# fengweie/UDA_CLR

Hardware: AMD Instinct MI355X
Metric: training images/sec (512x512, src+tgt) at 1/2/4/8 MI355X; val Dice vs ref (higher is better)
Workload: dtype f32

## Files before the change

uda_clr_amd/csrc/dwconv.hip:

```cpp
#include "dw_plan.h"

struct DwArgs {
    uda_src_t src;
    const float* w9c;
    int stride, dil, border_mode;
    int Ho, Wo;
    float* y;
    int64_t ldy;
    const float* dy;
    int64_t lddy;
    float* part;
    double* stats;
};

__device__ __forceinline__ float4 dw_transform(float4 v, const Xf4& xf, bool has_xf, int act) {
    float r[4] = {v.x, v.y, v.z, v.w};
#pragma unroll
    for (int j = 0; j < 4; ++j) {
        float u = r[j];
        if (has_xf) u = u * xf.sc[j] + xf.sh[j];
        r[j] = uda_act(u, act);
    }
    return make_float4(r[0], r[1], r[2], r[3]);
}

__global__ __launch_bounds__(256) void dwconv_fwd_kernel(DwArgs a) {
    __shared__ float red[2 * 1024];
    const int C = a.src.C, G = C >> 2, PP = 256 / G;
    const int tid = threadIdx.x, cg = tid % G, pl = tid / G;
    const bool active = pl < PP;
    const int H = a.src.H, W = a.src.W;
    const int64_t Pout = (int64_t)a.src.N * a.Ho * a.Wo;
    const int c0 = cg * 4;
    const bool has_xf = a.src.scale != nullptr;
    const int act = a.src.act;
    Xf4 xf;
    uda_load_xf4(xf, a.src.scale, a.src.shift, c0, C);
    float4 bval = make_float4(0.f, 0.f, 0.f, 0.f);
    if (a.border_mode == 1)
        bval = make_float4(uda_act(xf.sh[0], act), uda_act(xf.sh[1], act), uda_act(xf.sh[2], act), uda_act(xf.sh[3], act));
    float4 w[9];
#pragma unroll
    for (int t = 0; t < 9; ++t) w[t] = active ? uda_ld4(a.w9c + t * C + c0) : make_float4(0.f, 0.f, 0.f, 0.f);
    float4 s1 = make_float4(0.f, 0.f, 0.f, 0.f), s2 = s1;
    const int64_t base = (int64_t)blockIdx.x * (PP * DW_ITER_FWD);
    for (int it = 0; it < DW_ITER_FWD; ++it) {
        const int64_t po = base + (int64_t)it * PP + pl;
        if (!active || po >= Pout) continue;
        const int ow = (int)(po % a.Wo), oh = (int)((po / a.Wo) % a.Ho), n = (int)(po / ((int64_t)a.Wo * a.Ho));
        float4 acc = make_float4(0.f, 0.f, 0.f, 0.f);
#pragma unroll
        for (int kh = 0; kh < 3; ++kh) {
            const int ih = oh * a.stride + (kh - 1) * a.dil;
#pragma unroll
            for (int kw = 0; kw < 3; ++kw) {
                const int iw = ow * a.stride + (kw - 1) * a.dil;
                float4 u = bval;
                if (ih >= 0 && ih < H && iw >= 0 && iw < W)
                    u = dw_transform(uda_ld4(a.src.x + (((int64_t)n * H + ih) * W + iw) * a.src.ldx + c0), xf, has_xf, act);
                const float4 ww = w[kh * 3 + kw];
                acc.x += ww.x * u.x; acc.y += ww.y * u.y; acc.z += ww.z * u.z; acc.w += ww.w * u.w;
            }
        }
        uda_st4(a.y + po * a.ldy + c0, acc);
        s1.x += acc.x; s1.y += acc.y; s1.z += acc.z; s1.w += acc.w;
        s2.x += acc.x * acc.x; s2.y += acc.y * acc.y; s2.z += acc.z * acc.z; s2.w += acc.w * acc.w;
    }
    if (a.stats == nullptr) return;
    if (active) {
        uda_st4(&red[(pl * 2 + 0) * C + c0], s1);
        uda_st4(&red[(pl * 2 + 1) * C + c0], s2);
    }
    __syncthreads();
    double* dst = a.stats + (int64_t)(blockIdx.x % UDA_STAT_SLOTS) * 2 * C;
    for (int e = tid; e < 2 * C; e += 256) {
        float t = 0.f;
        for (int p = 0; p < PP; ++p) t += red[p * 2 * C + e];
        atomicAdd(&dst[e], (double)t);
    }
}

template <int S, int TH, int TW>
__device__ __forceinline__ void dw_stage_tile(float* tile, const float* xb, int64_t ldx, int H, int W, int gy0, int gx0, int IH, int IW, bool cok,
                                              const Xf4& xf, bool has_xf, int act, float4 bval, int pl, int cg) {
    constexpr int MAXL = (((TH - 1) * S + 5) * ((TW - 1) * S + 5) + 31) / 32;
    float4 v[MAXL];
    const int npix = IH * IW;
#pragma unroll
    for (int l = 0; l < MAXL; ++l) {
        const int idx = min(pl + 32 * l, npix - 1);
        const int iy = idx / IW, ix = idx - iy * IW;
        const int gy = min(max(gy0 + iy, 0), H - 1), gx = min(max(gx0 + ix, 0), W - 1);
        v[l] = uda_ld4(xb + ((int64_t)gy * W + gx) * ldx);
    }
#pragma unroll
    for (int l = 0; l < MAXL; ++l) {
        const int idx = pl + 32 * l;
        if (idx < npix) {
            const int iy = idx / IW, ix = idx - iy * IW;
            const int gy = gy0 + iy, gx = gx0 + ix;
            const bool in = cok && gy >= 0 && gy < H && gx >= 0 && gx < W;
            const float4 u = in ? dw_transform(v[l], xf, has_xf, act) : bval;
            uda_st4(&tile[idx * DWT_CB + cg * 4], u);
        }
    }
}

template <int S, int TH, int TW>
__global__ __launch_bounds__(256) void dwconv_fwd_tiled_kernel(DwArgs a, int tilesX, int tilesY) {
    extern __shared__ __attribute__((aligned(16))) float tile[];
    const int d = a.dil;
    const int IH = (TH - 1) * S + 2 * d + 1, IW = (TW - 1) * S + 2 * d + 1;
    const int C = a.src.C, H = a.src.H, W = a.src.W;
    const int tid = threadIdx.x, cg = tid & 7, pl = tid >> 3;
    int bt = blockIdx.x;
    const int tx = bt % tilesX; bt /= tilesX;
    const int ty = bt % tilesY;
    const int n = bt / tilesY;
    const int oy0 = ty * TH, ox0 = tx * TW;
    const int c0 = blockIdx.y * DWT_CB + cg * 4;
    const bool cok = c0 < C;
    const bool has_xf = a.src.scale != nullptr;
    const int act = a.src.act;
    Xf4 xf;
    uda_load_xf4(xf, a.src.scale, a.src.shift, c0, C);
    float4 bval = make_float4(0.f, 0.f, 0.f, 0.f);
    if (a.border_mode == 1)
        bval = make_float4(uda_act(xf.sh[0], act), uda_act(xf.sh[1], act), uda_act(xf.sh[2], act), uda_act(xf.sh[3], act));
    const int gy0 = oy0 * S - d, gx0 = ox0 * S - d;
    const float* xb = a.src.x + (int64_t)n * H * W * a.src.ldx + (cok ? c0 : 0);
    dw_stage_tile<S, TH, TW>(tile, xb, a.src.ldx, H, W, gy0, gx0, IH, IW, cok, xf, has_xf, act, bval, pl, cg);
    float4 w[9];
#pragma unroll
    for (int t = 0; t < 9; ++t) w[t] = cok ? uda_ld4(a.w9c + t * C + c0) : make_float4(0.f, 0.f, 0.f, 0.f);
    __syncthreads();
    float4 s1 = make_float4(0.f, 0.f, 0.f, 0.f), s2 = s1;
#pragma unroll
    for (int k = 0; k < (TH * TW) / 32; ++k) {
        const int op = pl + 32 * k;
        const int oy = op / TW, ox = op % TW;
        if (!cok || oy0 + oy >= a.Ho || ox0 + ox >= a.Wo) continue;
        float4 acc = make_float4(0.f, 0.f, 0.f, 0.f);
#pragma unroll
        for (int kh = 0; kh < 3; ++kh)
#pragma unroll
            for (int kw = 0; kw < 3; ++kw) {
                const float4 u = uda_ld4(&tile[((oy * S + kh * d) * IW + ox * S + kw * d) * DWT_CB + cg * 4]);
                const float4 ww = w[kh * 3 + kw];
                acc.x += ww.x * u.x; acc.y += ww.y * u.y; acc.z += ww.z * u.z; acc.w += ww.w * u.w;
            }
        uda_st4(a.y + (((int64_t)n * a.Ho + oy0 + oy) * a.Wo + ox0 + ox) * a.ldy + c0, acc);
        s1.x += acc.x; s1.y += acc.y; s1.z += acc.z; s1.w += acc.w;
        s2.x += acc.x * acc.x; s2.y += acc.y * acc.y; s2.z += acc.z * acc.z; s2.w += acc.w * acc.w;
    }
    if (a.stats == nullptr) return;
    __syncthreads();
    uda_st4(&tile[(pl * 2 + 0) * DWT_CB + cg * 4], s1);
    uda_st4(&tile[(pl * 2 + 1) * DWT_CB + cg * 4], s2);
    __syncthreads();
    if (tid < 2 * DWT_CB) {
        const int q = tid / DWT_CB, cl = tid % DWT_CB;
        const int c = blockIdx.y * DWT_CB + cl;
        if (c < C) {
            float t = 0.f;
            for (int p = 0; p < 32; ++p) t += tile[(p * 2 + q) * DWT_CB + cl];
            atomicAdd(&a.stats[((int64_t)(blockIdx.x % UDA_STAT_SLOTS) * 2 + q) * C + c], (double)t);
        }
    }
}

template <int S, int TH, int TW>
__global__ __launch_bounds__(256) void dwconv_wgrad_tiled_kernel(DwArgs a, int tilesX, int tilesY, double* sums) {
    extern __shared__ __attribute__((aligned(16))) float tile[];
    const int d = a.dil;
    const int IH = (TH - 1) * S + 2 * d + 1, IW = (TW - 1) * S + 2 * d + 1;
    const int C = a.src.C, H = a.src.H, W = a.src.W;
    const int tid = threadIdx.x, cg = tid & 7, pl = tid >> 3;
    int bt = blockIdx.x;
    const int tx = bt % tilesX; bt /= tilesX;
    const int ty = bt % tilesY;
    const int n = bt / tilesY;
    const int oy0 = ty * TH, ox0 = tx * TW;
    const int c0 = blockIdx.y * DWT_CB + cg * 4;
    const bool cok = c0 < C;
    const bool has_xf = a.src.scale != nullptr;
    const int act = a.src.act;
    Xf4 xf;
    uda_load_xf4(xf, a.src.scale, a.src.shift, c0, C);
    float4 bval = make_float4(0.f, 0.f, 0.f, 0.f);
    if (a.border_mode == 1)
        bval = make_float4(uda_act(xf.sh[0], act), uda_act(xf.sh[1], act), uda_act(xf.sh[2], act), uda_act(xf.sh[3], act));
    const int gy0 = oy0 * S - d, gx0 = ox0 * S - d;
    const float* xb = a.src.x + (int64_t)n * H * W * a.src.ldx + (cok ? c0 : 0);
    dw_stage_tile<S, TH, TW>(tile, xb, a.src.ldx, H, W, gy0, gx0, IH, IW, cok, xf, has_xf, act, bval, pl, cg);
    __syncthreads();
    float4 acc[9];
#pragma unroll
    for (int t = 0; t < 9; ++t) acc[t] = make_float4(0.f, 0.f, 0.f, 0.f);
    float4 gv[(TH * TW) / 32];
#pragma unroll
    for (int k = 0; k < (TH * TW) / 32; ++k) {
        const int op = pl + 32 * k;
        const int oy = min(oy0 + op / TW, a.Ho - 1), ox = min(ox0 + op % TW, a.Wo - 1);
        gv[k] = uda_ld4(a.dy + (((int64_t)n * a.Ho + oy) * a.Wo + ox) * a.lddy + (cok ? c0 : 0));
    }
#pragma unroll
    for (int k = 0; k < (TH * TW) / 32; ++k) {
        const int op = pl + 32 * k;
        const int oy = op / TW, ox = op % TW;
        if (!cok || oy0 + oy >= a.Ho || ox0 + ox >= a.Wo) continue;
        const float4 g = gv[k];
#pragma unroll
        for (int kh = 0; kh < 3; ++kh)
#pragma unroll
            for (int kw = 0; kw < 3; ++kw) {
                const float4 u = uda_ld4(&tile[((oy * S + kh * d) * IW + ox * S + kw * d) * DWT_CB + cg * 4]);
                float4& s = acc[kh * 3 + kw];
                s.x += g.x * u.x; s.y += g.y * u.y; s.z += g.z * u.z; s.w += g.w * u.w;
            }
    }
    __syncthreads();
#pragma unroll
    for (int t = 0; t < 9; ++t) uda_st4(&tile[(pl * 9 + t) * DWT_CB + cg * 4], acc[t]);
    __syncthreads();
    for (int e = tid; e < 9 * DWT_CB; e += 256) {
        const int t = e / DWT_CB, cl = e % DWT_CB;
        const int c = blockIdx.y * DWT_CB + cl;
        if (c < C) {
            float v = 0.f;
            for (int p = 0; p < 32; ++p) v += tile[(p * 9 + t) * DWT_CB + cl];
            atomicAdd(&sums[((int64_t)(blockIdx.x % UDA_STAT_SLOTS) * 9 + t) * C + c], (double)v);
        }
    }
}

__global__ void dw_wgrad_store_slots_kernel(const double* __restrict__ sums, int C, float* __restrict__ dw) {
    const int e = blockIdx.x * blockDim.x + threadIdx.x;
    if (e < 9 * C) {
        double v = 0.0;
        for (int k = 0; k < UDA_STAT_SLOTS; ++k) v += sums[(int64_t)k * 9 * C + e];
        dw[(e % C) * 9 + e / C] = (float)v;
    }
}

template <int S, int TH, int TW>
static int launch_dw_tiled(const DwArgs& a, const DwPlan& p, hipStream_t st) {
    auto fn = dwconv_fwd_tiled_kernel<S, TH, TW>;
    static size_t reserved = 0;
    if (p.lds > reserved && p.lds > 48 * 1024) {
        hipError_t e = hipFuncSetAttribute(reinterpret_cast<const void*>(fn), hipFuncAttributeMaxDynamicSharedMemorySize, (int)p.lds);
        if (e != hipSuccess) return uda_set_error("dwconv_fwd: cannot reserve %zu B of LDS: %s", p.lds, hipGetErrorString(e));
        reserved = p.lds;
    }
    hipLaunchKernelGGL(fn, dim3(p.gx, p.gy), dim3(256), p.lds, st, a, p.tilesX, p.tilesY);
    UDA_LAUNCH_CHECK("dwconv_fwd_tiled");
    return 0;
}

template <int S, int TH, int TW>
static int launch_dw_wgrad_tiled(const DwArgs& a, const DwPlan& p, double* sums, hipStream_t st) {
    auto fn = dwconv_wgrad_tiled_kernel<S, TH, TW>;
    static size_t reserved = 0;
    if (p.lds > reserved && p.lds > 48 * 1024) {
        hipError_t e = hipFuncSetAttribute(reinterpret_cast<const void*>(fn), hipFuncAttributeMaxDynamicSharedMemorySize, (int)p.lds);
        if (e != hipSuccess) return uda_set_error("dwconv_wgrad: cannot reserve %zu B of LDS: %s", p.lds, hipGetErrorString(e));
        reserved = p.lds;
    }
    hipLaunchKernelGGL(fn, dim3(p.gx, p.gy), dim3(256), p.lds, st, a, p.tilesX, p.tilesY, sums);
    UDA_LAUNCH_CHECK("dwconv_wgrad_tiled");
    return 0;
}

__global__ __launch_bounds__(256) void dwconv_dgrad_kernel(const float* __restrict__ dy, int64_t lddy,
                                                            const float* __restrict__ w9c, int C, int stride,
                                                            int dil, int N, int H, int W, int Ho, int Wo,
                                                            float* __restrict__ dx, int64_t lddx) {
    const int G = C >> 2;
    const int64_t total = (int64_t)N * H * W * G;
    for (int64_t e = (int64_t)blockIdx.x * blockDim.x + threadIdx.x; e < total; e += (int64_t)gridDim.x * blockDim.x) {
        const int cg = (int)(e % G);
        const int64_t p = e / G;
        const int iw = (int)(p % W), ih = (int)((p / W) % H), n = (int)(p / ((int64_t)W * H));
        const int c0 = cg * 4;
        float4 acc = make_float4(0.f, 0.f, 0.f, 0.f);
        if (stride == 2 && dil == 1) {
            const int khA = (ih & 1) ? 0 : 1, ohA = (ih + 1) >> 1, ohB = (ih - 1) >> 1;
            const int kwA = (iw & 1) ? 0 : 1, owA = (iw + 1) >> 1, owB = (iw - 1) >> 1;
            const int oha = (ih & 1) ? ohA : (ih >> 1), owa = (iw & 1) ? owA : (iw >> 1);
            const bool hA = oha < Ho, hB = (ih & 1) && ohB >= 0 && ohB < Ho;
            const bool wA = owa < Wo, wB = (iw & 1) && owB >= 0 && owB < Wo;
            const int r0 = min(oha, Ho - 1), r1 = min(max(ohB, 0), Ho - 1), q0 = min(owa, Wo - 1), q1 = min(max(owB, 0), Wo - 1);
            const float* base = dy + (int64_t)n * Ho * Wo * lddy + c0;
            const float4 g00 = uda_ld4(base + ((int64_t)r0 * Wo + q0) * lddy), g01 = uda_ld4(base + ((int64_t)r0 * Wo + q1) * lddy);
            const float4 g10 = uda_ld4(base + ((int64_t)r1 * Wo + q0) * lddy), g11 = uda_ld4(base + ((int64_t)r1 * Wo + q1) * lddy);
            const float4 w00 = uda_ld4(w9c + (khA * 3 + kwA) * C + c0), w01 = uda_ld4(w9c + (khA * 3 + 2) * C + c0);
            const float4 w10 = uda_ld4(w9c + (2 * 3 + kwA) * C + c0), w11 = uda_ld4(w9c + (2 * 3 + 2) * C + c0);
            const float k00 = (hA && wA) ? 1.f : 0.f, k01 = (hA && wB) ? 1.f : 0.f, k10 = (hB && wA) ? 1.f : 0.f, k11 = (hB && wB) ? 1.f : 0.f;
            acc.x = k00 * (w00.x * g00.x); acc.y = k00 * (w00.y * g00.y); acc.z = k00 * (w00.z * g00.z); acc.w = k00 * (w00.w * g00.w);
            acc.x += k01 * (w01.x * g01.x); acc.y += k01 * (w01.y * g01.y); acc.z += k01 * (w01.z * g01.z); acc.w += k01 * (w01.w * g01.w);
            acc.x += k10 * (w10.x * g10.x); acc.y += k10 * (w10.y * g10.y); acc.z += k10 * (w10.z * g10.z); acc.w += k10 * (w10.w * g10.w);
            acc.x += k11 * (w11.x * g11.x); acc.y += k11 * (w11.y * g11.y); acc.z += k11 * (w11.z * g11.z); acc.w += k11 * (w11.w * g11.w);
            uda_st4(dx + p * lddx + c0, acc);
            continue;
        }
#pragma unroll
        for (int kh = 0; kh < 3; ++kh) {
            const int nh = ih - (kh - 1) * dil;
            if (nh < 0 || nh % stride) continue;
            const int oh = nh / stride;
            if (oh >= Ho) continue;
#pragma unroll
            for (int kw = 0; kw < 3; ++kw) {
                const int nw = iw - (kw - 1) * dil;
                if (nw < 0 || nw % stride) continue;
                const int ow = nw / stride;
                if (ow >= Wo) continue;
                const float4 g = uda_ld4(dy + (((int64_t)n * Ho + oh) * Wo + ow) * lddy + c0);
                const float4 ww = uda_ld4(w9c + (kh * 3 + kw) * C + c0);
                acc.x += ww.x * g.x; acc.y += ww.y * g.y; acc.z += ww.z * g.z; acc.w += ww.w * g.w;
            }
        }
        uda_st4(dx + p * lddx + c0, acc);
    }
}

__global__ __launch_bounds__(256) void dwconv_wgrad_kernel(DwArgs a) {
    __shared__ float red[9 * 1024];
    const int C = a.src.C, G = C >> 2, PP = 256 / G;
    const int tid = threadIdx.x, cg = tid % G, pl = tid / G;
    const bool active = pl < PP;
    const int H = a.src.H, W = a.src.W;
    const int64_t Pout = (int64_t)a.src.N * a.Ho * a.Wo;
    const int c0 = cg * 4;
    const bool has_xf = a.src.scale != nullptr;
    const int act = a.src.act;
    Xf4 xf;
    uda_load_xf4(xf, a.src.scale, a.src.shift, c0, C);
    float4 bval = make_float4(0.f, 0.f, 0.f, 0.f);
    if (a.border_mode == 1)
        bval = make_float4(uda_act(xf.sh[0], act), uda_act(xf.sh[1], act), uda_act(xf.sh[2], act), uda_act(xf.sh[3], act));
    float4 acc[9];
#pragma unroll
    for (int t = 0; t < 9; ++t) acc[t] = make_float4(0.f, 0.f, 0.f, 0.f);
    const int64_t base = (int64_t)blockIdx.x * (PP * DW_ITER_RED);
// ... 156 lines not shown
#pragma unroll
    for (int t = 0; t < 9; ++t) uda_st4(&red[((pl * 9 + t) * CG + cl) * 4], acc[t]);
    __syncthreads();
    double* dst = sums + (int64_t)(blockIdx.x % UDA_STAT_SLOTS) * 9 * C;
    for (int e = tid; e < 9 * CG * 4; e += 256) {
        const int t = e / (CG * 4), cc = e - t * (CG * 4);
        const int c = blockIdx.y * CG * 4 + cc;
        if (c >= C) continue;
        float v = 0.f;
        for (int p = 0; p < PL; ++p) v += red[(p * 9 + t) * CG * 4 + cc];
        atomicAdd(&dst[t * C + c], (double)v);
    }
}

__global__ __launch_bounds__(256) void dwconv_cb_dgrad_kernel(const float* __restrict__ dy, int64_t lddy,
                                                               const float* __restrict__ w9c, int C, int stride, int dil,
                                                               int N, int H, int W, int Ho, int Wo,
                                                               float* __restrict__ dx, int64_t lddx, int lg) {
    const int CG = 1 << lg, PL = 256 >> lg, G = C >> 2;
    const int tid = threadIdx.x, cl = tid & (CG - 1), pl = tid >> lg;
    const int cg = blockIdx.y * CG + cl;
    const bool cok = cg < G;
    const int c0 = (cok ? cg : G - 1) * 4;
    const int64_t P = (int64_t)N * H * W;
    float4 w[9];
#pragma unroll
    for (int t = 0; t < 9; ++t) w[t] = uda_ld4(w9c + t * C + c0);
    const int64_t base = (int64_t)blockIdx.x * PL * DWB_ITER_FWD;
    for (int it = 0; it < DWB_ITER_FWD; ++it) {
        const int64_t p = base + (int64_t)it * PL + pl;
        if (p >= P) break;
        int n, ih, iw;
        dwb_pixel(p, W, H, n, ih, iw);
        int oh[3], ow[3];
        bool vh[3], vw[3];
#pragma unroll
        for (int k = 0; k < 3; ++k) {
            const int nh = ih - (k - 1) * dil, nw = iw - (k - 1) * dil;
            vh[k] = nh >= 0 && nh % stride == 0 && nh / stride < Ho;
            vw[k] = nw >= 0 && nw % stride == 0 && nw / stride < Wo;
            oh[k] = vh[k] ? nh / stride : 0;
            ow[k] = vw[k] ? nw / stride : 0;
        }
        const float* base_n = dy + (int64_t)n * Ho * Wo * lddy + c0;
        float4 g[9];
#pragma unroll
        for (int kh = 0; kh < 3; ++kh)
#pragma unroll
            for (int kw = 0; kw < 3; ++kw) g[kh * 3 + kw] = uda_ld4(base_n + ((int64_t)oh[kh] * Wo + ow[kw]) * lddy);
        float4 acc = make_float4(0.f, 0.f, 0.f, 0.f);
#pragma unroll
        for (int kh = 0; kh < 3; ++kh)
#pragma unroll
            for (int kw = 0; kw < 3; ++kw) {
                if (!(vh[kh] && vw[kw])) continue;
                const float4 ww = w[kh * 3 + kw], gg = g[kh * 3 + kw];
                acc.x += ww.x * gg.x; acc.y += ww.y * gg.y; acc.z += ww.z * gg.z; acc.w += ww.w * gg.w;
            }
        if (cok) uda_st4(dx + p * lddx + c0, acc);
    }
}

static_assert(DWF_AUTO == UDA_DW_AUTO && DWF_FLAT == UDA_DW_FLAT && DWF_TILED == UDA_DW_TILED && DWF_CB == UDA_DW_CB, "DwFamily is the ABI's UDA_DW_*");
static_assert(DW_FWD == UDA_DW_FWD && DW_DGRAD == UDA_DW_DGRAD && DW_WGRAD == UDA_DW_WGRAD, "DwOp is the ABI's UDA_DW_FWD ...");

static int dw_check(const uda_src_t* s, const char* who) {
    UDA_REQUIRE(s && s->x && uda_aligned16(s->x) && s->ldx % 4 == 0 && s->ldx >= s->C, "%s: bad src", who);
    UDA_REQUIRE((s->scale == nullptr) == (s->shift == nullptr), "%s: scale/shift must come together", who);
    UDA_REQUIRE(s->mask == nullptr, "%s: dropout masks are not supported on depthwise inputs", who);
    return 0;
}

#define DW_REQUIRE_PLAN(p, who, C, stride, dil) UDA_REQUIRE(!(p).error, "%s: C=%d, stride %d, dilation %d: %s", who, C, stride, dil, (p).error)

static DwArgs dw_args(const uda_src_t* src, const DwPlan& p, int stride, int dil, int border_mode) {
    DwArgs a = {};
    a.src = *src;
    a.stride = stride; a.dil = dil; a.border_mode = border_mode;
    a.Ho = p.Ho; a.Wo = p.Wo;
    return a;
}

static int dw_fwd_tiled(const DwArgs& a, const DwPlan& p, hipStream_t st) {
#define DW_LAUNCH(S_, TH_, TW_) if (p.S == S_ && p.TH == TH_ && p.TW == TW_) return launch_dw_tiled<S_, TH_, TW_>(a, p, st);
    DW_TILED_VARIANTS(DW_LAUNCH)
#undef DW_LAUNCH
    return uda_set_error("dwconv_fwd: no tiled kernel <%d, %d, %d>", p.S, p.TH, p.TW);
}

static int dw_wgrad_tiled(const DwArgs& a, const DwPlan& p, double* sums, hipStream_t st) {
#define DW_LAUNCH(S_, TH_, TW_) if (p.S == S_ && p.TH == TH_ && p.TW == TW_) return launch_dw_wgrad_tiled<S_, TH_, TW_>(a, p, sums, st);
    DW_TILED_VARIANTS(DW_LAUNCH)
#undef DW_LAUNCH
    return uda_set_error("dwconv_wgrad: no tiled kernel <%d, %d, %d>", p.S, p.TH, p.TW);
}

extern "C" uint64_t uda_dwconv_workspace_bytes(int64_t Pout, int C) {
    if (C < 4) return 0;
    uint64_t most = 0;
    for (int f = DWF_FLAT; f <= DWF_CB; ++f)
        if (C <= dw_cmax(DW_WGRAD, f)) {
            const uint64_t b = dw_wgrad_ws_bytes(f, Pout, C);
            if (b > most) most = b;
        }
    return most;
}

extern "C" int uda_dwconv_fwd(const uda_src_t* src, const float* w9c, int stride, int dil, int border_mode,
                              float* y, int64_t ldy, double* stats, int family, void* stream) {
    hipStream_t st = (hipStream_t)stream;
    if (int e = dw_check(src, "uda_dwconv_fwd")) return e;
    const DwPlan p = dw_plan(DW_FWD, src->N, src->H, src->W, src->C, stride, dil, family);
    DW_REQUIRE_PLAN(p, "uda_dwconv_fwd", src->C, stride, dil);
    UDA_REQUIRE(w9c && uda_aligned16(w9c) && y && uda_aligned16(y) && ldy % 4 == 0 && ldy >= src->C, "uda_dwconv_fwd: bad pointers");
    UDA_REQUIRE(border_mode == 0 || (border_mode == 1 && src->shift), "uda_dwconv_fwd: border_mode 1 needs shift");
    DwArgs a = dw_args(src, p, stride, dil, border_mode);
    a.w9c = w9c; a.y = y; a.ldy = ldy; a.stats = stats;
    if (p.family == DWF_TILED) return dw_fwd_tiled(a, p, st);
    if (p.family == DWF_CB) hipLaunchKernelGGL(dwconv_cb_fwd_kernel, dim3(p.gx, p.gy), dim3(256), 0, st, a, p.lg);
    else hipLaunchKernelGGL(dwconv_fwd_kernel, dim3(p.gx), dim3(256), 0, st, a);
    UDA_LAUNCH_CHECK(p.family == DWF_CB ? "dwconv_cb_fwd" : "dwconv_fwd");
    return 0;
}

extern "C" int uda_dwconv_dgrad(const float* dy, int64_t lddy, const float* w9c, int C, int stride, int dil,
                                int N, int H, int W, float* dx, int64_t lddx, int family, void* stream) {
    hipStream_t st = (hipStream_t)stream;
    UDA_REQUIRE(dy && w9c && dx && uda_aligned16(dy) && uda_aligned16(dx) && uda_aligned16(w9c), "uda_dwconv_dgrad: pointers must be 16-byte aligned");
    const DwPlan p = dw_plan(DW_DGRAD, N, H, W, C, stride, dil, family);
    DW_REQUIRE_PLAN(p, "uda_dwconv_dgrad", C, stride, dil);
    UDA_REQUIRE(lddy % 4 == 0 && lddx % 4 == 0 && lddy >= C && lddx >= C, "uda_dwconv_dgrad: lds must be multiples of 4, at least C");
    if (p.family == DWF_CB)
        hipLaunchKernelGGL(dwconv_cb_dgrad_kernel, dim3(p.gx, p.gy), dim3(256), 0, st, dy, lddy, w9c, C, stride, dil, N, H, W, p.Ho, p.Wo, dx, lddx, p.lg);
    else
        hipLaunchKernelGGL(dwconv_dgrad_kernel, dim3(p.gx), dim3(256), 0, st, dy, lddy, w9c, C, stride, dil, N, H, W, p.Ho, p.Wo, dx, lddx);
    UDA_LAUNCH_CHECK(p.family == DWF_CB ? "dwconv_cb_dgrad" : "dwconv_dgrad");
    return 0;
}

extern "C" int uda_dwconv_wgrad(const uda_src_t* src, const float* dy, int64_t lddy, int stride, int dil,
                                int border_mode, float* dw, float* workspace, uint64_t workspace_bytes, int family, void* stream) {
    hipStream_t st = (hipStream_t)stream;
    if (int e = dw_check(src, "uda_dwconv_wgrad")) return e;
    const int C = src->C;
    const DwPlan p = dw_plan(DW_WGRAD, src->N, src->H, src->W, C, stride, dil, family);
    DW_REQUIRE_PLAN(p, "uda_dwconv_wgrad", C, stride, dil);
    UDA_REQUIRE(dy && uda_aligned16(dy) && lddy % 4 == 0 && lddy >= C && dw, "uda_dwconv_wgrad: bad pointers");
    UDA_REQUIRE(border_mode == 0 || (border_mode == 1 && src->shift), "uda_dwconv_wgrad: border_mode 1 needs shift");
    UDA_REQUIRE(workspace && workspace_bytes >= uda_dwconv_workspace_bytes(p.Pout, C), "uda_dwconv_wgrad: workspace too small");
    DwArgs a = dw_args(src, p, stride, dil, border_mode);
    a.dy = dy; a.lddy = lddy;
    const dim3 store_grid(uda_cdiv(9 * C, 256));
    if (p.family == DWF_FLAT) {
        a.part = uda_wgp_part(workspace, 9 * C);
        uda_wgp_zero(workspace, 9 * C, st);
        hipLaunchKernelGGL(dwconv_wgrad_kernel, dim3(p.gx), dim3(256), 0, st, a);
        UDA_LAUNCH_CHECK("dwconv_wgrad");
        if (int e = uda_wgp_reduce(workspace, p.part_rows, 9 * C, st)) return e;
        hipLaunchKernelGGL(dw_wgrad_store_kernel, store_grid, dim3(256), 0, st, uda_wgp_sums(workspace), C, dw);
        UDA_LAUNCH_CHECK("dw_wgrad_store");
        return 0;
    }
    double* sums = reinterpret_cast<double*>(workspace);
    (void)hipMemsetAsync(sums, 0, (size_t)p.sum_slots * 9 * C * sizeof(double), st);
    if (p.family == DWF_CB) {
        hipLaunchKernelGGL(dwconv_cb_wgrad_kernel, dim3(p.gx, p.gy), dim3(256), 0, st, a, p.lg, sums);
        UDA_LAUNCH_CHECK("dwconv_cb_wgrad");
    } else if (int e = dw_wgrad_tiled(a, p, sums, st)) return e;
    hipLaunchKernelGGL(dw_wgrad_store_slots_kernel, store_grid, dim3(256), 0, st, sums, C, dw);
    UDA_LAUNCH_CHECK("dw_wgrad_store");
    return 0;
}

static const char* const DW_OP_NAME[3] = {"fwd", "dgrad", "wgrad"};
// ... 261 lines not shown
```

uda_clr_amd/csrc/igemm_conv.hip:

```cpp
#include <algorithm>
#include "common.h"
#include "conv_plan.h"

typedef float f32x16 __attribute__((ext_vector_type(16)));


#define IGC_MIN_WAVES(TM, TN, PIPE) ((PIPE) ? 2 : ((TM) * (TN) <= 3 ? 4 : 3))
template <int TM, int TN, int WM, int WN, bool PIPE = false, int XF = -1>
__global__ __launch_bounds__(256) void igemm_conv_kernel(ConvKArgs a) {
    constexpr int BM = 32 * TM * WM, BN = 32 * TN * WN;
    constexpr int A_IT = BM / 32, B_IT = BN / 32;
    constexpr int TILE = (BM + BN) * IG_LD;
    extern __shared__ __attribute__((aligned(16))) float smem[];

    const int tid = threadIdx.x, lane = tid & 63, wave = tid >> 6;
    const int wm = wave / WN, wn = wave % WN;
    const int lid = uda_xcd_remap(blockIdx.x, a.nMt * a.nNt);
    const int mt = lid / a.nNt, nt = lid % a.nNt;
    const int H = a.src.H, W = a.src.W, C = a.src.C;
    const int64_t P = (int64_t)a.src.N * H * W;
    const int64_t m0 = (int64_t)mt * BM;
    const int n0 = nt * BN;

    const int lrow = tid >> 3, kv = (tid & 7) * 4;
// ... 118 lines not shown
            t01 = f32x2{__builtin_amdgcn_fmed3f(t01.x, alo, ahi), __builtin_amdgcn_fmed3f(t01.y, alo, ahi)};
            t23 = f32x2{__builtin_amdgcn_fmed3f(t23.x, alo, ahi), __builtin_amdgcn_fmed3f(t23.y, alo, ahi)};
            if (masked) {
                const uint32_t mk = amask[i];
                t01 *= f32x2{(float)(mk & 0xffu), (float)((mk >> 8) & 0xffu)} * ms;
                t23 *= f32x2{(float)((mk >> 16) & 0xffu), (float)(mk >> 24)} * ms;
            }
            float v[4] = {t01.x, t01.y, t23.x, t23.y};
#pragma unroll
            for (int j = 0; j < 4; ++j)
                if (!(ok && (c_ci + j) < C)) v[j] = 0.f;
            uda_st4(&As[(lrow + 32 * i) * IG_LD + kv], make_float4(v[0], v[1], v[2], v[3]));
        }
#pragma unroll
        for (int i = 0; i < B_IT; ++i) uda_st4(&Bs[(lrow + 32 * i) * IG_LD + kv], breg[i]);
    };

    f32x16 acc[TM][TN];
#pragma unroll
    for (int i = 0; i < TM; ++i)
#pragma unroll
        for (int j = 0; j < TN; ++j)
#pragma unroll
            for (int r = 0; r < 16; ++r) acc[i][j][r] = 0.f;

    const int nchunks = (a.Ktot + IG_BK - 1) / IG_BK;
    const int arow = wm * TM * 32 + (lane & 31), brow = wn * TN * 32 + (lane & 31);
    const int koff = 4 * (lane >> 5);

    auto math = [&](const float* As, const float* Bs) {
#pragma unroll
        for (int g = 0; g < IG_BK / 8; ++g) {
            float4 af[TM], bf[TN];
#pragma unroll
            for (int i = 0; i < TM; ++i) af[i] = uda_ld4(&As[(arow + 32 * i) * IG_LD + g * 8 + koff]);
#pragma unroll
            for (int j = 0; j < TN; ++j) bf[j] = uda_ld4(&Bs[(brow + 32 * j) * IG_LD + g * 8 + koff]);
#pragma unroll
            for (int s = 0; s < 4; ++s) {
#pragma unroll
                for (int i = 0; i < TM; ++i) {
                    const float av = s == 0 ? af[i].x : s == 1 ? af[i].y : s == 2 ? af[i].z : af[i].w;
#pragma unroll
                    for (int j = 0; j < TN; ++j) {
                        const float bv = s == 0 ? bf[j].x : s == 1 ? bf[j].y : s == 2 ? bf[j].z : bf[j].w;
                        acc[i][j] = __builtin_amdgcn_mfma_f32_32x32x2f32(av, bv, acc[i][j], 0, 0, 0);
                    }
                }
            }
        }
    };
    float* As = smem;
    float* Bs = smem + BM * IG_LD;
    if constexpr (PIPE) {
        float* As1 = smem + TILE;
        float* Bs1 = As1 + BM * IG_LD;
        issue(0, R0);
        issue(1, R1);
        stage(R0, As, Bs);
        issue(2, R0);
        for (int c = 0; c < nchunks; c += 2) {
            __syncthreads();
            stage(R1, As1, Bs1);
            issue(c + 3, R1);
            math(As, Bs);
            __syncthreads();
            stage(R0, As, Bs);
            issue(c + 4, R0);
            if (c + 1 < nchunks) math(As1, Bs1);
        }
    } else {
        issue(0, R0);
        for (int c = 0; c < nchunks; ++c) {
            __syncthreads();
            stage(R0, As, Bs);
            __syncthreads();
            if (c + 1 < nchunks) issue(c + 1, R0);
            math(As, Bs);
        }
    }

    const int colb = n0 + wn * TN * 32 + (lane & 31);
    const bool vec_ok = uda_aligned16_dev(a.y) && (a.ldy & 3) == 0 && (!a.addend || (uda_aligned16_dev(a.addend) && (a.ld_add & 3) == 0));
    __syncthreads();
    float* patch = smem + wave * (32 * IG_LD);
    float s1[TN], s2[TN];
#pragma unroll
    for (int j = 0; j < TN; ++j) {
        s1[j] = 0.f;
        s2[j] = 0.f;
        const int col = colb + 32 * j;
        const bool cok = col < a.Cout;
        const float bv = (cok && a.bias) ? a.bias[col] : 0.f;
#pragma unroll
        for (int i = 0; i < TM; ++i) {
            const int64_t rbase = m0 + wm * TM * 32 + 32 * i;
#pragma unroll
            for (int r = 0; r < 16; ++r) {
                const int rl = (r & 3) + 8 * (r >> 2) + 4 * (lane >> 5);
                const float v = acc[i][j][r] + bv;
                if (cok && rbase + rl < P) {
                    s1[j] += v;
                    s2[j] += v * v;
                }
                if (vec_ok) {
                    patch[rl * IG_LD + (lane & 31)] = v;
                } else if (cok && rbase + rl < P) {
                    a.y[(rbase + rl) * a.ldy + col] = a.addend ? v + a.addend[(rbase + rl) * a.ld_add + col] : v;
                }
            }
            if (vec_ok) {
                const int cb = n0 + wn * TN * 32 + 32 * j + (lane & 7) * 4;
#pragma unroll
                for (int rq = 0; rq < 4; ++rq) {
                    const int rl = rq * 8 + (lane >> 3);
                    const int64_t row = rbase + rl;
                    float4 o = uda_ld4(&patch[rl * IG_LD + (lane & 7) * 4]);
                    if (row < P && cb < a.Cout) {
                        if (cb + 3 < a.Cout) {
                            if (a.addend) {
                                const float4 ad = uda_ld4(a.addend + row * a.ld_add + cb);
                                o.x += ad.x; o.y += ad.y; o.z += ad.z; o.w += ad.w;
                            }
                            uda_st4(a.y + row * a.ldy + cb, o);
                        } else {
                            const float ov[4] = {o.x, o.y, o.z, o.w};
                            for (int q = 0; q < 4; ++q)
                                if (cb + q < a.Cout) a.y[row * a.ldy + cb + q] = a.addend ? ov[q] + a.addend[row * a.ld_add + cb + q] : ov[q];
                        }
                    }
                }
            }
        }
    }
    if (a.stats) {
        __syncthreads();
        float* red = smem;
#pragma unroll
        for (int j = 0; j < TN; ++j) {
            const float t1 = s1[j] + __shfl_xor(s1[j], 32);
            const float t2 = s2[j] + __shfl_xor(s2[j], 32);
            if (lane < 32) {
                const int cl = wn * TN * 32 + 32 * j + lane;
                red[(wm * 2 + 0) * BN + cl] = t1;
                red[(wm * 2 + 1) * BN + cl] = t2;
            }
        }
        __syncthreads();
        double* dst = a.stats + (int64_t)(mt % UDA_STAT_SLOTS) * 2 * a.Cout;
        for (int e = tid; e < 2 * BN; e += 256) {
            const int qd = e / BN, cl = e % BN;
            if (n0 + cl < a.Cout) {
                float t = 0.f;
#pragma unroll
                for (int m = 0; m < WM; ++m) t += red[(m * 2 + qd) * BN + cl];
                atomicAdd(&dst[qd * a.Cout + n0 + cl], (double)t);
            }
        }
    }
}

__global__ void reduce_partials_kernel(const float* __restrict__ part, int nrows, int ncols,
                                       int rows_per_seg, double* __restrict__ out) {
    __shared__ double red[4][64];
    const int cl = threadIdx.x & 63, rg = threadIdx.x >> 6;
    const int col = blockIdx.x * 64 + cl;
    const int r0 = blockIdx.y * rows_per_seg;
    const int r1 = min(nrows, r0 + rows_per_seg);
    double s = 0.0;
    if (col < ncols)
        for (int r = r0 + rg; r < r1; r += 4) s += (double)part[(int64_t)r * ncols + col];
    red[rg][cl] = s;
    __syncthreads();
    if (rg == 0 && col < ncols) atomicAdd(&out[col], red[0][cl] + red[1][cl] + red[2][cl] + red[3][cl]);
}

int uda_reduce_partials(const float* part, int nrows, int ncols, double* out, hipStream_t st) {
    int segs = nrows / 64;
    if (segs < 1) segs = 1;
    if (segs > 64) segs = 64;
    const int rps = (nrows + segs - 1) / segs;
    dim3 grid(uda_cdiv(ncols, 64), uda_cdiv(nrows, rps));
    hipLaunchKernelGGL(reduce_partials_kernel, grid, dim3(256), 0, st, part, nrows, ncols, rps, out);
    UDA_LAUNCH_CHECK("reduce_partials");
    return 0;
}

static int check_src(const uda_src_t& s, const char* who) {
    UDA_REQUIRE(s.x && uda_aligned16(s.x), "%s: src.x must be 16-byte aligned", who);
    UDA_REQUIRE(s.ldx % 4 == 0 && s.ldx >= ((s.C + 3) / 4) * 4, "%s: src.ldx=%lld must be a multiple of 4 and >= round4(C=%d)",
                who, (long long)s.ldx, s.C);
    UDA_REQUIRE(s.N > 0 && s.H > 0 && s.W > 0 && s.C > 0, "%s: bad src dims", who);
    UDA_REQUIRE((s.scale == nullptr) == (s.shift == nullptr), "%s: scale/shift must come together", who);
    if (s.mask) UDA_REQUIRE(s.ldm % 4 == 0 && (reinterpret_cast<uintptr_t>(s.mask) & 3u) == 0 && s.ldm >= ((s.C + 3) / 4) * 4,
                            "%s: mask must be 4-byte aligned with ldm %% 4 == 0", who);
    return 0;
}

__global__ __launch_bounds__(256) void conv_cout1_kernel(ConvKArgs a) {
    const int lane = threadIdx.x & 63;
    const int64_t p = (int64_t)blockIdx.x * 4 + (threadIdx.x >> 6);
    const int H = a.src.H, W = a.src.W;
    const int64_t P = (int64_t)a.src.N * H * W;
    if (p >= P) return;
    const int pw = (int)(p % W), ph = (int)((p / W) % H);
    const int T = a.ksize * a.ksize;
    float acc = 0.f;
    for (int t = 0; t < T; ++t) {
        const int th = t / a.ksize;
        const int hh = ph + (th - a.cen) * a.dil, ww = pw + (t - th * a.ksize - a.cen) * a.dil;
        if (hh < 0 || hh >= H || ww < 0 || ww >= W) continue;
        const float* xr = a.src.x + (p + (int64_t)(hh - ph) * W + (ww - pw)) * a.src.ldx;
// ... 699 lines not shown
```

Before: 377.4.

## Specialize dwconv on dilation and store igemm epilogue directly via buffer ops

Depthwise conv forward and wgrad kernels gain a compile-time dilation parameter (1 or 2), so tile sizes and indexing become constants and the staging loop count fits the real halo. Separately, the implicit-GEMM conv epilogue no longer round-trips through an LDS patch with float4 stores. Each accumulator is now written straight to global memory with scalar raw buffer stores, using an out-of-range offset for masking, and the addend is read with buffer loads. This removes a __syncthreads and the LDS traffic, but the global stores become scalar, strided 32-lane column writes instead of coalesced 16-byte stores.

```diff
diff --git a/uda_clr_amd/csrc/dwconv.hip b/uda_clr_amd/csrc/dwconv.hip
--- a/uda_clr_amd/csrc/dwconv.hip
+++ b/uda_clr_amd/csrc/dwconv.hip
@@ -80,12 +80,12 @@
     }
 }
 
-template <int S, int TH, int TW>
-__device__ __forceinline__ void dw_stage_tile(float* tile, const float* xb, int64_t ldx, int H, int W, int gy0, int gx0, int IH, int IW, bool cok,
+template <int S, int TH, int TW, int D>
+__device__ __forceinline__ void dw_stage_tile(float* tile, const float* xb, int64_t ldx, int H, int W, int gy0, int gx0, bool cok,
                                               const Xf4& xf, bool has_xf, int act, float4 bval, int pl, int cg) {
-    constexpr int MAXL = (((TH - 1) * S + 5) * ((TW - 1) * S + 5) + 31) / 32;
+    constexpr int IH = (TH - 1) * S + 2 * D + 1, IW = (TW - 1) * S + 2 * D + 1, npix = IH * IW;
+    constexpr int MAXL = (npix + 31) / 32;
     float4 v[MAXL];
-    const int npix = IH * IW;
 #pragma unroll
     for (int l = 0; l < MAXL; ++l) {
         const int idx = min(pl + 32 * l, npix - 1);
@@ -106,11 +106,10 @@
     }
 }
 
-template <int S, int TH, int TW>
+template <int S, int TH, int TW, int D>
 __global__ __launch_bounds__(256) void dwconv_fwd_tiled_kernel(DwArgs a, int tilesX, int tilesY) {
     extern __shared__ __attribute__((aligned(16))) float tile[];
-    const int d = a.dil;
-    const int IH = (TH - 1) * S + 2 * d + 1, IW = (TW - 1) * S + 2 * d + 1;
+    constexpr int d = D, IW = (TW - 1) * S + 2 * D + 1;
     const int C = a.src.C, H = a.src.H, W = a.src.W;
     const int tid = threadIdx.x, cg = tid & 7, pl = tid >> 3;
     int bt = blockIdx.x;
@@ -129,7 +128,7 @@
         bval = make_float4(uda_act(xf.sh[0], act), uda_act(xf.sh[1], act), uda_act(xf.sh[2], act), uda_act(xf.sh[3], act));
     const int gy0 = oy0 * S - d, gx0 = ox0 * S - d;
     const float* xb = a.src.x + (int64_t)n * H * W * a.src.ldx + (cok ? c0 : 0);
-    dw_stage_tile<S, TH, TW>(tile, xb, a.src.ldx, H, W, gy0, gx0, IH, IW, cok, xf, has_xf, act, bval, pl, cg);
+    dw_stage_tile<S, TH, TW, D>(tile, xb, a.src.ldx, H, W, gy0, gx0, cok, xf, has_xf, act, bval, pl, cg);
     float4 w[9];
 #pragma unroll
     for (int t = 0; t < 9; ++t) w[t] = cok ? uda_ld4(a.w9c + t * C + c0) : make_float4(0.f, 0.f, 0.f, 0.f);
@@ -169,11 +168,10 @@
     }
 }
 
-template <int S, int TH, int TW>
+template <int S, int TH, int TW, int D>
 __global__ __launch_bounds__(256) void dwconv_wgrad_tiled_kernel(DwArgs a, int tilesX, int tilesY, double* sums) {
     extern __shared__ __attribute__((aligned(16))) float tile[];
-    const int d = a.dil;
-    const int IH = (TH - 1) * S + 2 * d + 1, IW = (TW - 1) * S + 2 * d + 1;
+    constexpr int d = D, IW = (TW - 1) * S + 2 * D + 1;
     const int C = a.src.C, H = a.src.H, W = a.src.W;
     const int tid = threadIdx.x, cg = tid & 7, pl = tid >> 3;
     int bt = blockIdx.x;
@@ -192,7 +190,7 @@
         bval = make_float4(uda_act(xf.sh[0], act), uda_act(xf.sh[1], act), uda_act(xf.sh[2], act), uda_act(xf.sh[3], act));
     const int gy0 = oy0 * S - d, gx0 = ox0 * S - d;
     const float* xb = a.src.x + (int64_t)n * H * W * a.src.ldx + (cok ? c0 : 0);
-    dw_stage_tile<S, TH, TW>(tile, xb, a.src.ldx, H, W, gy0, gx0, IH, IW, cok, xf, has_xf, act, bval, pl, cg);
+    dw_stage_tile<S, TH, TW, D>(tile, xb, a.src.ldx, H, W, gy0, gx0, cok, xf, has_xf, act, bval, pl, cg);
     __syncthreads();
     float4 acc[9];
 #pragma unroll
@@ -243,9 +241,9 @@
     }
 }
 
-template <int S, int TH, int TW>
+template <int S, int TH, int TW, int D>
 static int launch_dw_tiled(const DwArgs& a, const DwPlan& p, hipStream_t st) {
-    auto fn = dwconv_fwd_tiled_kernel<S, TH, TW>;
+    auto fn = dwconv_fwd_tiled_kernel<S, TH, TW, D>;
     static size_t reserved = 0;
     if (p.lds > reserved && p.lds > 48 * 1024) {
         hipError_t e = hipFuncSetAttribute(reinterpret_cast<const void*>(fn), hipFuncAttributeMaxDynamicSharedMemorySize, (int)p.lds);
@@ -257,9 +255,9 @@
     return 0;
 }
 
-template <int S, int TH, int TW>
+template <int S, int TH, int TW, int D>
 static int launch_dw_wgrad_tiled(const DwArgs& a, const DwPlan& p, double* sums, hipStream_t st) {
-    auto fn = dwconv_wgrad_tiled_kernel<S, TH, TW>;
+    auto fn = dwconv_wgrad_tiled_kernel<S, TH, TW, D>;
     static size_t reserved = 0;
     if (p.lds > reserved && p.lds > 48 * 1024) {
         hipError_t e = hipFuncSetAttribute(reinterpret_cast<const void*>(fn), hipFuncAttributeMaxDynamicSharedMemorySize, (int)p.lds);
@@ -582,14 +580,14 @@
 }
 
 static int dw_fwd_tiled(const DwArgs& a, const DwPlan& p, hipStream_t st) {
-#define DW_LAUNCH(S_, TH_, TW_) if (p.S == S_ && p.TH == TH_ && p.TW == TW_) return launch_dw_tiled<S_, TH_, TW_>(a, p, st);
+#define DW_LAUNCH(S_, TH_, TW_) if (p.S == S_ && p.TH == TH_ && p.TW == TW_) return a.dil == 1 ? launch_dw_tiled<S_, TH_, TW_, 1>(a, p, st) : launch_dw_tiled<S_, TH_, TW_, 2>(a, p, st);
     DW_TILED_VARIANTS(DW_LAUNCH)
 #undef DW_LAUNCH
     return uda_set_error("dwconv_fwd: no tiled kernel <%d, %d, %d>", p.S, p.TH, p.TW);
 }
 
 static int dw_wgrad_tiled(const DwArgs& a, const DwPlan& p, double* sums, hipStream_t st) {
-#define DW_LAUNCH(S_, TH_, TW_) if (p.S == S_ && p.TH == TH_ && p.TW == TW_) return launch_dw_wgrad_tiled<S_, TH_, TW_>(a, p, sums, st);
+#define DW_LAUNCH(S_, TH_, TW_) if (p.S == S_ && p.TH == TH_ && p.TW == TW_) return a.dil == 1 ? launch_dw_wgrad_tiled<S_, TH_, TW_, 1>(a, p, sums, st) : launch_dw_wgrad_tiled<S_, TH_, TW_, 2>(a, p, sums, st);
     DW_TILED_VARIANTS(DW_LAUNCH)
 #undef DW_LAUNCH
     return uda_set_error("dwconv_wgrad: no tiled kernel <%d, %d, %d>", p.S, p.TH, p.TW);
diff --git a/uda_clr_amd/csrc/igemm_conv.hip b/uda_clr_amd/csrc/igemm_conv.hip
--- a/uda_clr_amd/csrc/igemm_conv.hip
+++ b/uda_clr_amd/csrc/igemm_conv.hip
@@ -224,52 +224,64 @@
 
     const int colb = n0 + wn * TN * 32 + (lane & 31);
     const bool vec_ok = uda_aligned16_dev(a.y) && (a.ldy & 3) == 0 && (!a.addend || (uda_aligned16_dev(a.addend) && (a.ld_add & 3) == 0));
-    __syncthreads();
-    float* patch = smem + wave * (32 * IG_LD);
+    const int wm_u = __builtin_amdgcn_readfirstlane(wm);
+    const int half4 = 4 * (lane >> 5);
+    const int ldy4 = (int)a.ldy * 4, lda4 = (int)a.ld_add * 4;
+    constexpr int EP_OOB = 0x7ffffff0;
     float s1[TN], s2[TN];
 #pragma unroll
     for (int j = 0; j < TN; ++j) {
         s1[j] = 0.f;
         s2[j] = 0.f;
-        const int col = colb + 32 * j;
-        const bool cok = col < a.Cout;
-        const float bv = (cok && a.bias) ? a.bias[col] : 0.f;
-#pragma unroll
-        for (int i = 0; i < TM; ++i) {
-            const int64_t rbase = m0 + wm * TM * 32 + 32 * i;
-#pragma unroll
-            for (int r = 0; r < 16; ++r) {
-                const int rl = (r & 3) + 8 * (r >> 2) + 4 * (lane >> 5);
-                const float v = acc[i][j][r] + bv;
-                if (cok && rbase + rl < P) {
-                    s1[j] += v;
-                    s2[j] += v * v;
+    }
+#pragma unroll
+    for (int i = 0; i < TM; ++i) {
+        const int64_t rbase = m0 + wm_u * TM * 32 + 32 * i;
+        const int rows_left = (int)min((int64_t)32, P - rbase);
+        const bool any = rows_left > 0;
+        const __amdgpu_buffer_rsrc_t yres = __builtin_amdgcn_make_buffer_rsrc(
+            a.y + (any ? rbase : 0) * a.ldy, 0, (vec_ok && any) ? ((rows_left - 1) * (int)a.ldy + a.Cout) * 4 : 0, 0x00020000);
+        const __amdgpu_buffer_rsrc_t adres = __builtin_amdgcn_make_buffer_rsrc(
+            const_cast<float*>(a.addend ? a.addend + (any ? rbase : 0) * a.ld_add : a.y), 0,
+            (vec_ok && any && a.addend) ? ((rows_left - 1) * (int)a.ld_add + a.Cout) * 4 : 0, 0x00020000);
+#pragma unroll
+        for (int j = 0; j < TN; ++j) {
+            const int col = colb + 32 * j;
+            const bool cok = col < a.Cout;
+            const float bv = (cok && a.bias) ? a.bias[col] : 0.f;
+            if (vec_ok) {
+                float ad[16];
+#pragma unroll
+                for (int r = 0; r < 16; ++r) ad[r] = 0.f;
+                if (a.addend) {
+#pragma unroll
+                    for (int r = 0; r < 16; ++r) {
+                        const int rl = (r & 3) + 8 * (r >> 2);
+                        const bool ok = cok && rl + half4 < rows_left;
+                        ad[r] = __builtin_bit_cast(float, __builtin_amdgcn_raw_buffer_load_b32(adres, ok ? half4 * lda4 + col * 4 : EP_OOB, rl * lda4, 0));
+                    }
                 }
-                if (vec_ok) {
-                    patch[rl * IG_LD + (lane & 31)] = v;
-                } else if (cok && rbase + rl < P) {
-                    a.y[(rbase + rl) * a.ldy + col] = a.addend ? v + a.addend[(rbase + rl) * a.ld_add + col] : v;
+#pragma unroll
+                for (int r = 0; r < 16; ++r) {
+                    const int rl = (r & 3) + 8 * (r >> 2);
+                    const bool ok = cok && rl + half4 < rows_left;
+                    const float v = acc[i][j][r] + bv;
+                    if (ok) {
+                        s1[j] += v;
+                        s2[j] += v * v;
+                    }
+                    __builtin_amdgcn_raw_buffer_store_b32(__builtin_bit_cast(unsigned, a.addend ? v + ad[r] : v), yres, ok ? half4 * ldy4 + col * 4 : EP_OOB,
+                                                          rl * ldy4, 0);
                 }
-            }
-            if (vec_ok) {
-                const int cb = n0 + wn * TN * 32 + 32 * j + (lane & 7) * 4;
-#pragma unroll
-                for (int rq = 0; rq < 4; ++rq) {
-                    const int rl = rq * 8 + (lane >> 3);
-                    const int64_t row = rbase + rl;
-                    float4 o = uda_ld4(&patch[rl * IG_LD + (lane & 7) * 4]);
-                    if (row < P && cb < a.Cout) {
-                        if (cb + 3 < a.Cout) {
-                            if (a.addend) {
-                                const float4 ad = uda_ld4(a.addend + row * a.ld_add + cb);
-                                o.x += ad.x; o.y += ad.y; o.z += ad.z; o.w += ad.w;
-                            }
-                            uda_st4(a.y + row * a.ldy + cb, o);
-                        } else {
-                            const float ov[4] = {o.x, o.y, o.z, o.w};
-                            for (int q = 0; q < 4; ++q)
-                                if (cb + q < a.Cout) a.y[row * a.ldy + cb + q] = a.addend ? ov[q] + a.addend[row * a.ld_add + cb + q] : ov[q];
-                        }
+            } else {
+#pragma unroll
+                for (int r = 0; r < 16; ++r) {
+                    const int rl = (r & 3) + 8 * (r >> 2) + half4;
+                    const float v = acc[i][j][r] + bv;
+                    if (cok && rbase + rl < P) {
+                        s1[j] += v;
+                        s2[j] += v * v;
+                        a.y[(rbase + rl) * a.ldy + col] = a.addend ? v + a.addend[(rbase + rl) * a.ld_add + col] : v;
                     }
                 }
             }
```

New measurement: 378.1, median of 2. Within noise of the previous version (+0.2%).
